# marcusrussi/approximateNN

Hardware: AMD Instinct MI355X
Metric: queries/sec, N=10M d=128 k=10 Q=10k float (query(): hash + candidate gather + L2 + top-k + refine) (higher is better)
Workload: dtype f32; 1 GPU; cfg3: N=10000000 d=128 k=10 tries=10 Q=10000/step float; streams=1, d_short=20, L1=6006, P1=4096, L2=110, P2=64, sum_par_maxes=286

## Files before the change

### approximatenn_amd/csrc/ann_host.hip

```cpp
#include <hip/hip_fp16.h>
#include <hip/hip_runtime.h>
#include <math.h>
#include <stdio.h>
#include <stdlib.h>
#include <string.h>
#include <time.h>

#include <algorithm>
#include <limits>
#include <mutex>
#include <vector>

#include "../../include/algg.h"
#include "../../include/ann_hip.h"
#include "../../include/gpu_comp.h"
#include "ann_hostpool.h"
#include "ann_precomp_kernels.h"
#include "ann_query_kernels.h"
#include "ann_probe_kernels.h"
#include "ann_recall_kernels.h"
#include "ann_exact_kernels.h"
#include "ann_filter_kernels.h"
#include "ann_tag_kernels.h"
#include "ann_kq_kernels.h"
// ... 202 lines not shown
static T *dev_alloc(size_t count) {
  void *p = NULL;
  HIPCHECK(hipMalloc(&p, (count ? count : 1) * sizeof(T)));
  return (T *)p;
}

static int device_cus() {
  static int cus[64] = {0};
  int dev = 0;
  if (hipGetDevice(&dev) != hipSuccess || dev < 0 || dev >= 64) return 256;
  if (!cus[dev]) {
    hipDeviceProp_t prop;
    cus[dev] = hipGetDeviceProperties(&prop, dev) == hipSuccess && prop.multiProcessorCount > 0 ? prop.multiProcessorCount : 256;
  }
  return cus[dev];
}

static unsigned grid_for(size_t work, unsigned block, unsigned cap = 1u << 20) {
  size_t g = (work + block - 1) / block;
  if (g < 1) g = 1;
  if (g > cap) g = cap;
  return (unsigned)g;
}

#define ANN_NCOUNTERS (8 + 64 * 8)
struct EventPair {
  hipEvent_t a, b;
};

struct annhip_workspace {
  DevBuf codes, cand_d, cand_i, nvt, nvo, top_i, top_d, flist, xids, xd, r2i, r2d, out_i, out_d;
  DevBuf pbits;
  DevBuf sorted;
  u32 *d_fcount = NULL;
  void release() {
    DevBuf *bufs[] = {&codes, &cand_d, &cand_i, &nvt, &nvo, &top_i, &top_d, &flist, &xids, &xd, &r2i, &r2d, &out_i, &out_d, &pbits, &sorted};
    for (DevBuf *b : bufs) b->release();
    if (d_fcount) HIPCHECK(hipFree(d_fcount));
    d_fcount = NULL;
  }
};

#ifdef USE_FLOAT
#define ANNHIP_ROWS_NARROW ANNHIP_ROWS_F16
#define ANN_NARROW_WHAT "binary16"
#else
#define ANNHIP_ROWS_NARROW ANNHIP_ROWS_F32
#define ANN_NARROW_WHAT "binary32"
#endif

struct annhip_index {
  size_t n = 0, k = 0, d = 0, ds = 0, lo = 0, hi = 0;
  int T = 0;
  FT *d_points = NULL;
  bool own_points = false;
  std::vector<u32 *> d_tabs;
  std::vector<uint2 *> d_segs;
  std::vector<uint4 *> d_segx;
  int use_seg = 1;
  std::vector<TryInfo> h_tries;
  TryInfo *d_tries = NULL;
  u32 *d_graph = NULL;
  FT *d_means = NULL, *d_bases = NULL;
  FT *d_graph_dists = NULL;
  u32 L1 = 0, P1 = 0, Lc1 = 0, L2 = 0, P2 = 0, Lc2 = 0;
  size_t sum_pm = 0;
  hipStream_t stream = 0;
  annhip_workspace ws;
  DevBuf io_y, io_ids, io_dist;
// ... 855 lines not shown
        constexpr bool FU = decltype(fu)::value, RG = decltype(rg)::value;
        using RT = typename decltype(rt)::type;
        allow_lds(stage1_select_kernel<D, SG, FU, RT, RG>, smem);
        for (size_t a = 0; a < Q; a += per) {
          QParams Pp = P;
          Pp.q0 = (u32)a, Pp.qn = (u32)std::min(per, Q - a);
          hipLaunchKernelGGL((stage1_select_kernel<D, SG, FU, RT, RG>), dim3(std::min<unsigned>(Pp.qn, max_grid)), dim3(64 * W), smem,
                             s, Pp, kq, y, alias, codes, K1, cap, runs_used, cand_d, cand_i, nvt, nvo, F, cand_key);
        }
      };
      auto launch = [&](auto sg, auto fu) {
        if constexpr (sel_regs_layout<decltype(dd)::value>()) {
          if (regs) return launch_sel(sg, fu, std::true_type{});
        } else if (regs) {
          die("launch_stage1: register selection chosen for a layout without one");
        }
        launch_sel(sg, fu, std::false_type{});
      };
      if (use_seg == 2) launch(Int<2>{}, std::false_type{});
      else if (use_seg && F.enabled == 1) launch(Int<1>{}, std::true_type{});
      else if (use_seg) launch(Int<1>{}, std::false_type{});
      else if (F.enabled == 1) launch(Int<0>{}, std::true_type{});
      else launch(Int<0>{}, std::false_type{});
    });
  });
  HIPCHECK(hipGetLastError());
  if (prof) s1_prof_end(ix, ev, Q, nvo, s);
  if (ix) ix->s1_launches += 1;
}

#ifdef USE_FLOAT
static void launch_prune_rescore(annhip_index *ix, const QParams &P, size_t Q, const FT *y, int kp, const FT *pre_d,
                                 const u32 *pre_i, const u32 *nvt, u32 *nvo, u32 *top_i, FT *top_d, u32 *fl, u32 *d_fcount,
                                 hipStream_t s) {
  if (!Q) return;
  if (kp < P.k + 1 || kp > ANN_PRUNE_KMAX || P.k + 1 > 32) die("launch_prune_rescore: preselection size out of range");
  PruneArgs A = {};
  A.points = P.points, A.y = y, A.pre_d = pre_d, A.pre_i = pre_i, A.nv_tot = nvt, A.nv_own = nvo;
  A.top_id = top_i, A.top_dist = top_d, A.flist = fl, A.fcount = d_fcount;
  A.exact_total = ix->d_rows + 2, A.uncertified = ix->d_rows + 4;
  A.E = ix->prune_E;
  A.n = P.n, A.Q = (u32)Q, A.L1 = P.L1, A.P1 = P.P1;
  A.d = P.d, A.k = P.k, A.Kp = kp;
  const dim3 grid((unsigned)((Q + ANN_PRUNE_WAVES - 1) / ANN_PRUNE_WAVES)), block(64 * ANN_PRUNE_WAVES);
  with_value(QueryLayouts{}, layout_code(P.d), [&](auto dc) {
    constexpr int D = decltype(dc)::value;
    if constexpr (D != 0 && !OcCode<D>::GEN) hipLaunchKernelGGL(prune_rescore_kernel<D>, grid, block, 0, s, A);
    else die("launch_prune_rescore: no register layout for this row length");
  });
  HIPCHECK(hipGetLastError());
}
#endif

static void launch_codes_probe(const QParams &P, size_t Q, const FT *y, u32 *codes, unsigned char *pbits, int pb, hipStream_t s,
                               u32 *zero_me = NULL) {
  const int wpb = ANN_PROBE_WPB;
  const size_t items = Q * (size_t)P.T;
  if (!items) return;
  if (pb < 1 || pb > P.ds || P.ds > 31) die("launch_codes_probe: pair bits outside 1..d_short");
  if (d_is_fast(P.d) && (size_t)P.d * sizeof(FT) <= 512 && env().codes_lpq) {
    const size_t smem = sizeof(FT) * ((size_t)P.ds + 1) * P.d + sizeof(u32) * ANN_WAVE * ANN_LPQ_WAVES +
                        sizeof(UB) * (size_t)P.ds * ANN_WAVE;
    const dim3 grid((unsigned)((Q + ANN_WAVE - 1) / ANN_WAVE), (unsigned)P.T);
    with_value(Pow2Layouts{}, layout_code(P.d, false), [&](auto dd) {
      constexpr int D = decltype(dd)::value;
      if constexpr (D > 0 && D * sizeof(FT) <= 512) {
        allow_lds(codes_probe_lpq_kernel<D>, smem);
        hipLaunchKernelGGL(codes_probe_lpq_kernel<D>, grid, dim3(64 * ANN_LPQ_WAVES), smem, s, P, (int)Q, y, codes, zero_me, pb, pbits);
      }
    });
  } else if (d_is_fast(P.d)) {
    const size_t smem = sizeof(FT) * (size_t)P.ds * P.d;
    const dim3 grid((unsigned)((Q + ANN_CODES_QPB - 1) / ANN_CODES_QPB), (unsigned)P.T);
// ... 136 lines not shown
  const unsigned block = len <= 128 ? 128 : 256;
  const unsigned flat = live_rows ? split : 0;
  const dim3 grid = live_rows ? dim3((unsigned)std::min<size_t>(nq * split, 512)) : dim3((unsigned)nq, split);
  with_value(QueryLayouts{}, layout_code(P.d), [&](auto dd) {
    with_rows(P, [&](auto rt) {
      constexpr int D = decltype(dd)::value;
      using RT = typename decltype(rt)::type;
      allow_lds(row_dists_kernel<D, MODE, RT>, smem);
      hipLaunchKernelGGL((row_dists_kernel<D, MODE, RT>), grid, dim3(block), smem, s, P, kq, y, alias, codes, qidx, xbase, len,
                         top_i, top_d, ids, dist, rows_done, live_rows, (u32)nq, chunk, live_off, flat);
    });
  });
  HIPCHECK(hipGetLastError());
}

static void launch_exact_select(u32 L, u32 len, u32 in_stride, int k, size_t nq, u32 *ids, FT *dist,
                                const u32 *qidx, u32 xbase, u32 *out_i, FT *out_d, int ostride, int ooff,
                                hipStream_t s, const u32 *live_rows = NULL, size_t *out64 = NULL, unsigned max_block = 1024,
                                u32 live_off = 0, TieArgs tie = TieArgs{NULL, NULL, 0, NULL, 0}) {
  if (!nq) return;
  const int lk = ann_lg(L);
  unsigned npairs = 8u << (lk > 4 ? lk - 4 : 0);
  if (live_rows) max_block = std::min(max_block, 256u);
  unsigned block = npairs >= max_block ? max_block : ((npairs + 63) / 64) * 64;
  if (block < 64) block = 64;
  const size_t row_smem = (size_t)len * (sizeof(FT) + sizeof(u32));
  const unsigned grid = live_rows ? (unsigned)std::min<size_t>(nq, 128) : (unsigned)nq;
  const bool in_lds = row_smem <= env().lds_row_max;
  const u32 Pn = (u32)1 << lk;
  int nw = 0;
  if ((tie.cand_d || tie.derive) && env().tie && L >= 16 && tie.K1 == k + 1 && tie.K1 <= ANN_WAVE && (u32)k <= Pn)
    nw = Pn <= 4096 ? 1 : Pn <= 8192 ? 2 : Pn <= 16384 ? 4 : 0;
  size_t tie_smem = nw ? ann_tie_lds_bytes(nw) : 0;
  if (nw && !tie.cand_d) tie_smem += ann_tie_derive_bytes(Pn);
  if (tie_smem > 150 * 1024) nw = 0;
  if (!nw) tie = TieArgs{NULL, NULL, 0, NULL, 0}, tie_smem = 0;
  const size_t smem = std::max(in_lds ? row_smem : (size_t)0, tie_smem);
  auto launch = [&](auto lds, auto nwc) {
    constexpr bool LDS = decltype(lds)::value;
    constexpr int NW = decltype(nwc)::value;
    allow_lds((exact_select_kernel<LDS, NW>), smem);
    hipLaunchKernelGGL((exact_select_kernel<LDS, NW>), dim3(grid), dim3(block), smem, s, L, len, in_stride, k, ids, dist, qidx,
                       xbase, out_i, out_d, ostride, ooff, live_rows, (u32)nq, out64, live_off, tie);
  };
  with_value(Ints<0, 1, 2, 4>{}, nw, [&](auto nwc) {
    if (in_lds) launch(std::true_type{}, nwc);
    else launch(std::false_type{}, nwc);
  });
  HIPCHECK(hipGetLastError());
}

template <typename IdOut>
static void launch_stage2_fused(const QParams &P, size_t Q, const FT *y, int alias, u32 xbase, size_t nq, const u32 *top_i,
                                const FT *top_d, IdOut *out_ids, FT *out_d, unsigned long long *rows_ctr, hipStream_t s) {
  if (!nq) return;
  size_t smem = sizeof(Key) * (size_t)P.k + 3 * sizeof(u32) * (size_t)P.Lc2 + 16;
  smem = (smem + 15) & ~(size_t)15;
  smem += sizeof(FT) * (size_t)P.Lc2;
  smem = (smem + 15) & ~(size_t)15;
  if (d_needs_lds_row(P.d)) smem += sizeof(FT) * (size_t)P.d * 3;
  with_value(QueryLayouts{}, layout_code(P.d), [&](auto dd) {
    with_rows(P, [&](auto rt) {
      constexpr int D = decltype(dd)::value;
      using RT = typename decltype(rt)::type;
      allow_lds((stage2_fused_kernel<D, IdOut, RT>), smem);
      hipLaunchKernelGGL((stage2_fused_kernel<D, IdOut, RT>), dim3((unsigned)nq), dim3(env().s2_threads), smem, s, P, (int)Q, y,
                         alias, top_i, top_d, P.Lc2, out_ids, out_d, rows_ctr, xbase);
// ... 36 lines not shown
        if (filter) {
          allow_lds((stage2_filter_kernel<D, TT, RT>), smem);
          hipLaunchKernelGGL((stage2_filter_kernel<D, TT, RT>), dim3((unsigned)nq), dim3(64 * W), smem, s, P, (int)Q, y, alias,
                             top_i, top_d, filter, P2, K1, cap, out, out_d, fl, d_fcount, exact_total, rows_ctr, xbase);
          return;
        }
        allow_lds((stage2_select_kernel<D, TT, RT>), smem);
        hipLaunchKernelGGL((stage2_select_kernel<D, TT, RT>), dim3((unsigned)nq), dim3(64 * W), smem, s, P, (int)Q, y, alias,
                           top_i, top_d, P2, K1, cap, out, out_d, fl, d_fcount, exact_total, rows_ctr, xbase);
      };
      if (out64) launch(out64);
      else launch(out32);
    });
  });
  HIPCHECK(hipGetLastError());
  if (P.fixed) return true;
  const size_t R = std::min(nq, chunk);
  u32 *ri = (u32 *)r2i.need(sizeof(u32) * R * P.Lc2);
  FT *rd = (FT *)r2d.need(sizeof(FT) * R * P.Lc2);
  for (size_t p0 = 0; p0 < nq; p0 += R) {
    const size_t np = std::min(R, nq - p0);
    launch_rows<MODE_GRAPH>(P, Q, y, alias, NULL, fl + p0, 0, np, P.Lc2, top_i, top_d, ri, rd, rows_ctr, s, d_fcount, (u32)p0);
    launch_exact_select(P.L2, P.Lc2, P.Lc2, P.k, np, ri, rd, fl + p0, 0, out32, out_d, P.k, 0, s, d_fcount, out64, 1024,
                        (u32)p0);
  }
  return true;
}

static long finalize_and_fallback(annhip_index *ix, const QParams &P, size_t Q, const FT *y, int alias,
                                  const u32 *codes, int mode, const FT *cand_d, const u32 *cand_i,
                                  const u32 *nvt, u32 *top_i, FT *top_d, int ostride, int ooff, DevBuf &flist,
                                  DevBuf &xids, DevBuf &xd, u32 *d_fcount, unsigned long long *rows_done,
                                  unsigned long long *exact_total, bool device_driven, hipStream_t s, size_t qstride = 0,
                                  bool prefinalized = false) {
  const int K1 = P.k + 1;
  unsigned long long *tie_ctr = ix ? ix->d_rows + 3 : NULL;
  const TieArgs tie0 = cand_d ? TieArgs{cand_d, cand_i, K1, tie_ctr, 0} : TieArgs{NULL, NULL, K1, tie_ctr, 1};
  u32 nflag = 0;
  u32 *fl = (u32 *)flist.need(sizeof(u32) * Q);
  const size_t row_bytes = (size_t)P.Lc1 * (sizeof(FT) + sizeof(u32));
  size_t chunk = env().exact_bytes / (row_bytes ? row_bytes : 1);
  if (chunk < 1) chunk = 1;
  if (mode == 0) {
    if (!prefinalized) {
      zero_u32_kernel<<<1, 1, 0, s>>>(d_fcount);
      hipLaunchKernelGGL(finalize1_kernel, dim3(grid_for(Q, 256, 1u << 30)), dim3(256), 0, s, (int)Q, P.k, K1, P.L1,
                         P.P1, cand_d, cand_i, nvt, top_i, top_d, ostride, ooff, fl, d_fcount, exact_total);
      HIPCHECK(hipGetLastError());
    }
    if (device_driven && Q <= 8 * chunk) {
      const size_t R = std::min(Q, chunk);
      u32 *ids = (u32 *)xids.need(sizeof(u32) * R * P.Lc1);
      FT *dist = (FT *)xd.need(sizeof(FT) * R * P.Lc1);
      for (size_t p0 = 0; p0 < Q; p0 += R) {
        const size_t nq = std::min(R, Q - p0);
        launch_rows<MODE_TABLE>(P, Q, y, alias, codes, fl + p0, 0, nq, P.Lc1, NULL, NULL, ids, dist, rows_done, s, d_fcount,
                                (u32)p0, qstride);
        launch_exact_select(P.L1, P.Lc1, P.Lc1, P.k, nq, ids, dist, fl + p0, 0, top_i, top_d, ostride, ooff, s, d_fcount,
                            NULL, 1024, (u32)p0, tie0);
      }
      return -1;
    }
    HIPCHECK(hipMemcpyAsync(&nflag, d_fcount, sizeof(u32), hipMemcpyDeviceToHost, s));
    HIPCHECK(hipStreamSynchronize(s));
  } else {
    nflag = (u32)Q;
    if (exact_total) {
      unsigned long long add = Q, cur = 0;
      HIPCHECK(hipMemcpyAsync(&cur, exact_total, sizeof cur, hipMemcpyDeviceToHost, s));
      HIPCHECK(hipStreamSynchronize(s));
// ... 131 lines not shown
      FusedTail F{1, P.Lc2, ids_dev, out_d, fl, ws.d_fcount, ix->d_rows + 2, NULL, NULL};
      cand_d = (FT *)ws.cand_d.need(sizeof(FT) * Q * K1);
      cand_i = (u32 *)ws.cand_i.need(sizeof(u32) * Q * K1);
      launch_stage1(ix, P, Q, y, alias, codes, cand_d, cand_i, NULL, nvo, s, ix->h_tries, ix->use_seg, F);
      seg_mark(ix, marks, s);
      unsigned long long *rows_ctr = ix->profile == 1 ? ix->d_rows + 8 : NULL;
      u32 *xi = (u32 *)ws.xids.need(sizeof(u32) * Q * P.Lc1);
      FT *xd = (FT *)ws.xd.need(sizeof(FT) * Q * P.Lc1);
      launch_rows<MODE_TABLE>(P, Q, y, alias, codes, fl, 0, Q, P.Lc1, NULL, NULL, xi, xd, rows_ctr, s, ws.d_fcount);
      launch_exact_select(P.L1, P.Lc1, P.Lc1, k, Q, xi, xd, fl, 0, top_i, top_d, k, 0, s, ws.d_fcount, NULL, 1024, 0,
                          TieArgs{cand_d, cand_i, K1, ix->d_rows + 3, 0});
      seg_mark(ix, marks, s);
      u32 *r2i = (u32 *)ws.r2i.need(sizeof(u32) * Q * P.Lc2);
      FT *r2d = (FT *)ws.r2d.need(sizeof(FT) * Q * P.Lc2);
      launch_rows<MODE_GRAPH>(P, Q, y, alias, NULL, fl, 0, Q, P.Lc2, top_i, top_d, r2i, r2d, rows_ctr, s, ws.d_fcount);
      seg_mark(ix, marks, s);
      launch_exact_select(P.L2, P.Lc2, P.Lc2, k, Q, r2i, r2d, fl, 0, NULL, out_d, k, 0, s, ws.d_fcount, ids_dev);
      seg_mark(ix, marks, s);
      seg_mark(ix, marks, s);
      if (marks) ix->seg_used.push_back(marks_store);
      ix->queries += (double)Q;
      return -1;
    }
  }
  bool prefinalized = false;
#ifdef USE_FLOAT
  if (pruned) {
    const int kp = ix->prune_kp;
    FT *pre_d = (FT *)ws.cand_d.need(sizeof(FT) * Q * kp);
    u32 *pre_i = (u32 *)ws.cand_i.need(sizeof(u32) * Q * kp);
    nvt = (u32 *)ws.nvt.need(sizeof(u32) * Q);
    u32 *nvo = (u32 *)ws.nvo.need(sizeof(u32) * Q);
    u32 *fl = (u32 *)ws.flist.need(sizeof(u32) * Q);
    prefinalized = true;
    if (!fcount_zeroed) zero_u32_kernel<<<1, 1, 0, s>>>(ws.d_fcount);
    QParams Pn = P;
    Pn.points_h = ix->d_points_h;
    EventPair ev;
    if (ix->profile) ev = s1_prof_begin(ix, s);
    launch_stage1(ix, Pn, Q, y, alias, codes, pre_d, pre_i, nvt, nvo, s, ix->h_tries, ix->use_seg,
                  FusedTail{0, 0, NULL, NULL, NULL, NULL, NULL, NULL, NULL}, NULL, 1, env().s1_slots, qstride, kp, false);
    launch_prune_rescore(ix, P, Q, y, kp, pre_d, pre_i, nvt, nvo, top_i, top_d, fl, ws.d_fcount, s);
    if (ix->profile) s1_prof_end(ix, ev, Q, nvo, s);
  } else
#endif
  if (mode == 0) {
    cand_d = (FT *)ws.cand_d.need(sizeof(FT) * Q * K1);
    cand_i = (u32 *)ws.cand_i.need(sizeof(u32) * Q * K1);
    nvt = (u32 *)ws.nvt.need(sizeof(u32) * Q);
    u32 *nvo = (u32 *)ws.nvo.need(sizeof(u32) * Q);
    u32 *fl = (u32 *)ws.flist.need(sizeof(u32) * Q);
    prefinalized = env().fin_tail != 0;
    if (prefinalized && !fcount_zeroed) zero_u32_kernel<<<1, 1, 0, s>>>(ws.d_fcount);
    launch_stage1(ix, P, Q, y, alias, codes, cand_d, cand_i, nvt, nvo, s, ix->h_tries, ix->use_seg,
                  FusedTail{prefinalized ? 2 : 0, 0, NULL, NULL, fl, ws.d_fcount, ix->d_rows + 2, top_i, top_d}, NULL, 1,
                  env().s1_slots, qstride);
  }
  seg_mark(ix, marks, s);
  unsigned long long *rows_ctr = ix->profile == 1 ? ix->d_rows + 8 : NULL;
  long nflag = finalize_and_fallback(ix, P, Q, y, alias, codes, mode, cand_d, cand_i, nvt, top_i, top_d, k, 0,
                                     ws.flist, ws.xids, ws.xd, ws.d_fcount, rows_ctr, ix->d_rows + 2, true, s, qstride,
                                     prefinalized);
  seg_mark(ix, marks, s);
  FT *out_d = dists_dev ? reinterpret_cast<FT *>(dists_dev) : (FT *)ws.out_d.need(sizeof(FT) * Q * k);
  if (ix->lo == 0 && ix->hi == ix->n && P.Lc2 <= 1024 && env().tail != 0) {
    launch_stage2_fused<size_t>(P, Q, y, alias, 0, Q, top_i, top_d, ids_dev, out_d, rows_ctr, s);
    seg_mark(ix, marks, s);
    seg_mark(ix, marks, s);
    seg_mark(ix, marks, s);
    if (marks) ix->seg_used.push_back(marks_store);
    ix->queries += (double)Q;
    return nflag;
  }
  if (ix->lo == 0 && ix->hi == ix->n && env().tail != 0 &&
      stage2_select_with_fallback(P, Q, y, alias, 0, Q, top_i, top_d, NULL, ids_dev, out_d, ws.flist, ws.d_fcount, ws.r2i,
                                  ws.r2d, ix->d_rows + 2, rows_ctr, s)) {
    seg_mark(ix, marks, s);
    seg_mark(ix, marks, s);
    seg_mark(ix, marks, s);
    if (marks) ix->seg_used.push_back(marks_store);
    ix->queries += (double)Q;
    return nflag;
  }
  u32 *out_i = (u32 *)ws.out_i.need(sizeof(u32) * Q * k);
  const size_t row_bytes = (size_t)P.Lc2 * (sizeof(FT) + sizeof(u32));
  size_t chunk = ((size_t)2 << 30) / row_bytes;
  if (chunk < 1) chunk = 1;
  for (size_t q0 = 0; q0 < Q; q0 += chunk) {
    const size_t nq = std::min(chunk, Q - q0);
    u32 *r2i = (u32 *)ws.r2i.need(sizeof(u32) * nq * P.Lc2);
    FT *r2d = (FT *)ws.r2d.need(sizeof(FT) * nq * P.Lc2);
    launch_rows<MODE_GRAPH>(P, Q, y, alias, NULL, NULL, (u32)q0, nq, P.Lc2, top_i, top_d, r2i, r2d, rows_ctr, s);
    if (q0 + chunk >= Q) seg_mark(ix, marks, s);
    launch_exact_select(P.L2, P.Lc2, P.Lc2, k, nq, r2i, r2d, NULL, (u32)q0, out_i, out_d, k, 0, s);
  }
// ... 2050 lines not shown
```

### approximatenn_amd/csrc/ann_prune_kernels.h

```cpp
#pragma once
#include "ann_rerank_kernels.h"

#define ANN_PRUNE_WAVES 4
#define ANN_PRUNE_KMAX 64

struct PruneArgs {
  const FT *points, *y;
  const FT *pre_d;
  const u32 *pre_i;
  const u32 *nv_tot;
  u32 *nv_own;
  u32 *top_id;
  FT *top_dist;
  u32 *flist, *fcount;
  unsigned long long *exact_total, *uncertified;
  double E;
  u32 n, Q, L1, P1;
  int d, k, Kp;
};

template <int D>
__global__ __launch_bounds__(64 * ANN_PRUNE_WAVES) void prune_rescore_kernel(PruneArgs A) {
  __shared__ Key s_keys[ANN_PRUNE_WAVES][ANN_PRUNE_KMAX], s_sorted[ANN_PRUNE_WAVES][ANN_PRUNE_KMAX];
  __shared__ u32 s_ids[ANN_PRUNE_WAVES][ANN_PRUNE_KMAX];
  constexpr int C = RowChunks<D>::C;
  const int lane = lane_id(), w = threadIdx.x >> 6;
  const int d = A.d, k = A.k, K1 = A.k + 1, Kp = A.Kp;
  const u32 q = __builtin_amdgcn_readfirstlane(blockIdx.x * ANN_PRUNE_WAVES + w);
  if (q >= A.Q) return;
  Key *keys = s_keys[w], *sorted = s_sorted[w];
  u32 *ids = s_ids[w];
  const u32 myid = lane < Kp ? A.pre_i[(size_t)q * Kp + lane] : ANN_ID_NONE;
  const bool real = myid < A.n;
  const u64 rm = __ballot(real);
  const int m = __builtin_popcountll(rm);
  if (real) ids[mask_rank(rm)] = myid;
  const ExLanes<D> ln(d, lane);
  VT a[C];
  const FT *yq = A.y + (size_t)q * d;
#pragma unroll
  for (int c = 0; c < C; c++) {
    if constexpr (D > 0) a[c] = reinterpret_cast<const VT *>(yq)[ln.p + c * ln.oc];
    else a[c] = oc_load_chunk<D, false>(yq, ln.p + c * ln.oc, d);
  }
  wave_lds_sync();
  const FT *__restrict__ points = A.points;
  auto load = [&](VT(&b)[C], int r0, u32 &id) {
    const int r = r0 + ln.g;
    id = ids[(ln.valid && r < m) ? r : r0];
    const FT *rp = points + (size_t)id * d;
#pragma unroll
    for (int c = 0; c < C; c++) {
      if constexpr (D > 0) b[c] = reinterpret_cast<const VT *>(rp)[ln.p + c * ln.oc];
      else b[c] = oc_load_chunk<D, false>(rp, ln.p + c * ln.oc, d);
    }
  };
  auto score = [&](const VT(&b)[C], int r0, u32 id) {
    const FT dist = ex_reduce<D>(a, b, ln.oc, ln.p, d);
    if (ln.valid && r0 + ln.g < m && ln.p == 0) keys[r0 + ln.g] = key_make(dist, id);
  };
  if (m) {
    VT b0[C], b1[C];
    u32 i0 = 0, i1 = 0;
    load(b0, 0, i0);
    for (int r0 = 0; r0 < m; r0 += 2 * ln.rpw) {
      const int r1 = r0 + ln.rpw, r2 = r1 + ln.rpw;
      if (r1 < m) load(b1, r1, i1);
      score(b0, r0, i0);
      if (r1 < m) {
        if (r2 < m) load(b0, r2, i0);
        score(b1, r1, i1);
      }
    }
  }
  wave_lds_sync();
  const Key me = keys[lane < m ? lane : 0];
  int rank = 0;
  for (int t = 0; t < m; t++) rank += key_less(keys[t], me) ? 1 : 0;
  if (lane < m) sorted[rank] = me;
  wave_lds_sync();
  const int me_cnt = m < K1 ? m : K1;
  bool cert = m < Kp;
  if (!cert && m >= K1) {
    const double B = (double)A.pre_d[(size_t)q * Kp + Kp - 1];
    const double tau = (double)key_dist(sorted[K1 - 1]);
    const double g1 = 1.0 - 0x1p-16;
    const double r = sqrt(B * g1) - A.E;
    if (B >= 0x1p-100 && r > 0.0) {
      const double LB = (r * r) * g1 * (1.0 - 0x1p-40);
      if (LB > tau) cert = true;
    }
  }
  bool bad = me_cnt < k;
  for (int t = lane; t + 1 < me_cnt; t += ANN_WAVE)
    if (ft_bits(key_dist(sorted[t])) == ft_bits(key_dist(sorted[t + 1]))) bad = true;
  if (me_cnt >= k && !(key_dist(sorted[k - 1]) < ft_inf())) bad = true;
  if (A.L1 > A.P1 && A.nv_tot[q] >= A.P1) bad = true;
  if (!cert || __ballot(bad) != 0) {
    if (lane == 0) {
      A.flist[atomicAdd(A.fcount, 1u)] = q;
      if (A.exact_total) atomicAdd(A.exact_total, 1ull);
      if (!cert && A.uncertified) atomicAdd(A.uncertified, 1ull);
    }
  } else {
    for (int t = lane; t < k; t += ANN_WAVE) {
      A.top_id[(size_t)q * k + t] = key_id(sorted[t]);
      A.top_dist[(size_t)q * k + t] = key_dist(sorted[t]);
    }
  }
  if (lane == 0 && A.nv_own) A.nv_own[q] = (A.nv_own[q] + 1) / 2 + (u32)m;
}

__global__ __launch_bounds__(256) void prune_rowerr_kernel(size_t rows, int d, const FT *__restrict__ points,
                                                           const RN *__restrict__ narrow, unsigned long long *out) {
  const int lane = lane_id();
  const size_t wave = ((size_t)blockIdx.x * blockDim.x + threadIdx.x) >> 6, waves = ((size_t)gridDim.x * blockDim.x) >> 6;
  double worst = 0;
  bool broken = false;
  for (size_t r = wave; r < rows; r += waves) {
    double acc = 0;
    for (int z = lane; z < d; z += ANN_WAVE) {
      const double df = (double)points[r * d + z] - (double)narrow[r * d + z];
      acc += df * df;
    }
#pragma unroll
    for (int s = 32; s >= 1; s >>= 1) acc += __shfl_xor(acc, s);
    if (!(acc < __builtin_inf())) broken = true;
    else if (acc > worst) worst = acc;
  }
  if (lane == 0) {
    atomicMax(out, (unsigned long long)__builtin_bit_cast(unsigned long long, worst));
    if (broken) atomicAdd(out + 1, 1ull);
  }
}
```

### approximatenn_amd/csrc/ann_query_kernels.h

```cpp
#pragma once
#include <type_traits>

#include "ann_device.h"
#include "ann_tie.h"

#ifndef ANN_ROWS_INFLIGHT
#define ANN_ROWS_INFLIGHT 1
#endif

struct TryInfo {
  const u32 *tab;
  const uint2 *seg;
  const uint4 *segx;
  u32 pm;
  u32 off;
  u32 end;
  u32 magic;
};

struct QParams {
  const FT *points;
  const TryInfo *tries;
  const u32 *graph;
  const FT *means;
// ... 14 lines not shown
#define ANN_S1_PREFETCH_NARROW 3
#endif
#ifndef ANN_S1_PREFETCH_OC
#define ANN_S1_PREFETCH_OC 2
#endif

template <bool NT>
__device__ __forceinline__ VT load_row_chunk(const VT *p) {
  if constexpr (NT) {
    typedef FT native_vec __attribute__((ext_vector_type(ANN_VEC)));
    native_vec v = __builtin_nontemporal_load(reinterpret_cast<const native_vec *>(p));
    return __builtin_bit_cast(VT, v);
  } else {
    return *p;
  }
}

template <typename RT>
__device__ __forceinline__ const RT *q_rows(const QParams &P) {
  if constexpr (std::is_same<RT, FT>::value) return P.points;
  else return P.points_h;
}
template <typename RT, bool NT>
__device__ __forceinline__ typename RowRaw<RT>::T load_row_raw(const RT *row, int ci) {
  if constexpr (std::is_same<RT, FT>::value) {
    return load_row_chunk<NT>(reinterpret_cast<const VT *>(row) + ci);
  } else {
    typedef typename RowRaw<RT>::T R;
    const R *p = reinterpret_cast<const R *>(row) + ci;
    if constexpr (NT) return __builtin_nontemporal_load(p);
    else return *p;
  }
}

template <int D, bool NT, typename RT>
__device__ __forceinline__ typename RowRaw<RT>::T oc_load_chunk(const RT *row, int ci, int d) {
  if constexpr (OcCode<D>::UA) {
    typename RowRaw<RT>::T v;
    RT *o = reinterpret_cast<RT *>(&v);
#pragma unroll
    for (int j = 0; j < ANN_VEC; j++) {
      const int z = ci * ANN_VEC + j;
      o[j] = z < d ? (NT ? __builtin_nontemporal_load(row + z) : row[z]) : (RT)0;
    }
    return v;
  } else {
    return load_row_raw<RT, NT>(row, ci);
  }
}
template <int D>
__device__ __forceinline__ int oc_tree_len(int d) { return OcCode<D>::UA ? d : 0; }

#define ANN_CODES_QPB 64
template <int D>
__global__ __launch_bounds__(256) void codes_kernel(QParams P, int Q, const FT *__restrict__ y,
                                                    u32 *__restrict__ codes, u32 *__restrict__ zero_me) {
  extern __shared__ __attribute__((aligned(16))) unsigned char smem[];
  if (zero_me && blockIdx.x == 0 && blockIdx.y == 0 && threadIdx.x == 0) *zero_me = 0;
  const int lane = lane_id(), w = threadIdx.x >> 6, wpb = blockDim.x >> 6;
  if constexpr (D > 0) {
    typedef RowLay<D> L;
    const int t = blockIdx.y;
    const int q0 = blockIdx.x * ANN_CODES_QPB, q1 = min(Q, q0 + ANN_CODES_QPB);
    VT *rows = reinterpret_cast<VT *>(smem);
    const VT *src = reinterpret_cast<const VT *>(P.bases + (size_t)t * P.ds * D);
    for (int i = threadIdx.x; i < P.ds * (D / ANN_VEC); i += blockDim.x) rows[i] = src[i];
// ... 404 lines not shown
    }
    const Key key = key_make(v, id);
    const bool pass = act && z == 0 && key_less(key, S.tau);
    const u64 mm = __ballot(pass);
    if (mm) {
      if (pass) S.kbuf[S.kcnt + mask_rank(mm)] = key;
      S.kcnt += __popcll(mm);
      if (S.kcnt + rpw > S.cap) sel_shrink(S);
    }
  }
}

template <int D, typename RT = FT, typename ST = SelState>
__device__ __forceinline__ void gather_select(const QParams &P, const u32 *list, int cnt, int alias, u32 x,
                                              const VT (&a)[RowChunks<D>::C],
                                              const FT *yq, FT *scratch, ST &S, const FT *yrow = NULL) {
  const int lane = lane_id();
  const RT *rows = q_rows<RT>(P);
  typedef typename RowRaw<RT>::T RR;
  if constexpr (D > 0) {
    typedef RowLay<D> L;
    constexpr int PF = std::is_same<RT, FT>::value ? ANN_S1_PREFETCH : ANN_S1_PREFETCH_NARROW;
    const int p = lane % L::LPR, g = lane / L::LPR;
    RR buf[PF][L::C];
    u32 idb[PF];
#pragma unroll
    for (int s = 0; s < PF; s++) {
      const int first = s * L::RPW;
      idb[s] = 0;
      if (first < cnt) {
        idb[s] = list[first + g < cnt ? first + g : first];
        const RT *rp = rows + (size_t)(idb[s] - P.lo) * D;
#pragma unroll
        for (int c = 0; c < L::C; c++) buf[s][c] = load_row_raw<RT, true>(rp, p + c * L::LPR);
      }
    }
    for (int base = 0; base < cnt; base += PF * L::RPW) {
#pragma unroll
      for (int s = 0; s < PF; s++) {
        const int cur = base + s * L::RPW;
        if (cur < cnt) {
          const u32 id = idb[s];
          const bool act = cur + g < cnt && !(alias && id == x);
          const FT dist = row_reduce<D, ROW_SQDIFF>(a, buf[s]);
          const int nb = cur + PF * L::RPW;
          if (nb < cnt) {
            idb[s] = list[nb + g < cnt ? nb + g : nb];
            const RT *rp = rows + (size_t)(idb[s] - P.lo) * D;
#pragma unroll
            for (int c = 0; c < L::C; c++) buf[s][c] = load_row_raw<RT, true>(rp, p + c * L::LPR);
          }
          const Key key = key_make(dist, id);
          const bool pass = act && p == 0 && key_less(key, S.tau);
          sel_offer(S, key, pass, L::RPW);
        }
      }
    }
  } else if constexpr (OcCode<D>::FOLD > 0) {
    const FoldPlan fp(P.d);
    gather_fold<OcCode<D>::FOLD, RT>(P, fp, list, cnt, alias, x, yrow, S);
  } else if constexpr (D < 0 && !OcCode<D>::GEN) {
    constexpr int C = OcCode<D>::C, OC = OcCode<D>::OC;
    constexpr int PF = ANN_S1_PREFETCH_OC;
    const OcLanes<D> ol(P.d, lane);
    const int oc = ol.oc, rpw = ol.rpw, g = ol.g, p = ol.p;
    RR buf[PF][C];
    u32 idb[PF];
#pragma unroll
    for (int s = 0; s < PF; s++) {
      const int first = s * rpw;
      idb[s] = 0;
      if (first < cnt) {
        idb[s] = list[(ol.valid && first + g < cnt) ? first + g : first];
        const RT *rp = rows + (size_t)(idb[s] - P.lo) * P.d;
#pragma unroll
        for (int c = 0; c < C; c++) buf[s][c] = oc_load_chunk<D, OcCode<D>::NT_ROWS>(rp, p + c * oc, P.d);
      }
    }
    for (int base = 0; base < cnt; base += PF * rpw) {
#pragma unroll
      for (int s = 0; s < PF; s++) {
        const int cur = base + s * rpw;
        if (cur < cnt) {
// ... 41 lines not shown
    u32 id;
    if (j < (u32)k) {
      id = key_id(top[j]);
      t_dist[j] = key_dist(top[j]);
    } else {
      const u32 parent = key_id(top[j / k - 1]), z = j % k;
      id = parent < P.n ? P.graph[(size_t)parent * k + z] : (P.graph[z] | P.n);
      const bool ok = id < P.n && !(alias && id == x) && id >= P.lo && id < P.hi;
      if (ok) {
        const u32 pos = atomicAdd(cnt2p, 1u);
        t_slot[pos] = j;
        t_gid[pos] = id;
      } else {
        t_dist[j] = ft_inf();
      }
    }
    t_ids[j] = id;
  }
  __syncthreads();
  const int cnt2 = (int)*cnt2p;
  if constexpr (D > 0) {
    typedef RowLay<D> L;
    constexpr int U = (ANN_ROWS_INFLIGHT / L::C) > 0 ? (ANN_ROWS_INFLIGHT / L::C) : 1;
    const int p = lane % L::LPR, g = lane / L::LPR;
    for (int base0 = w * L::RPW; base0 < cnt2; base0 += W * L::RPW * U) {
      RR b[U][L::C];
#pragma unroll
      for (int u = 0; u < U; u++) {
        const int r = base0 + u * W * L::RPW + g;
        if (base0 + u * W * L::RPW < cnt2) {
          const u32 id = t_gid[r < cnt2 ? r : base0];
          const RT *rp = rows + (size_t)(id - P.lo) * D;
#pragma unroll
          for (int c = 0; c < L::C; c++) b[u][c] = load_row_raw<RT, true>(rp, p + c * L::LPR);
        }
      }
#pragma unroll
      for (int u = 0; u < U; u++) {
        const int r = base0 + u * W * L::RPW + g;
        if (base0 + u * W * L::RPW < cnt2) {
          const FT dist = row_reduce<D, ROW_SQDIFF>(a, b[u]);
          if (r < cnt2 && p == 0) t_dist[t_slot[r]] = dist;
        }
      }
    }
  } else if constexpr (D < 0 && !OcCode<D>::GEN) {
    constexpr int C = OcCode<D>::C, OC = OcCode<D>::OC;
    constexpr int U = C <= 2 ? 4 : 2;
    const OcLanes<D> ol(P.d, lane);
    const int oc = ol.oc, rpw = ol.rpw, g = ol.g, p = ol.p;
    for (int base0 = w * rpw; base0 < cnt2; base0 += W * rpw * U) {
      RR b[U][C];
#pragma unroll
      for (int u = 0; u < U; u++) {
        const int r = base0 + u * W * rpw + g;
        if (base0 + u * W * rpw < cnt2) {
          const u32 id = t_gid[(ol.valid && r < cnt2) ? r : base0];
          const RT *rp = rows + (size_t)(id - P.lo) * P.d;
#pragma unroll
          for (int c = 0; c < C; c++) b[u][c] = oc_load_chunk<D, OcCode<D>::NT_ROWS>(rp, p + c * oc, P.d);
        }
      }
#pragma unroll
      for (int u = 0; u < U; u++) {
        const int r = base0 + u * W * rpw + g;
        if (base0 + u * W * rpw < cnt2) {
          const FT dist = row_reduce_oc<C, ROW_SQDIFF, OC>(a, b[u], oc, p, oc_tree_len<D>(P.d));
// ... 760 lines not shown
          id = parent < P.n ? P.graph[(size_t)parent * k + z] : (P.graph[z] | P.n);
        }
      }
      if (!DIST_ONLY) ids_row[j] = id;
      if (given) {
        dist_row[j] = top_dist[(size_t)x * P.k + j];
      } else {
        const bool own = id < P.n && !(alias && id == x) && id >= P.lo && id < P.hi;
        if (own) {
          const u32 pos = atomicAdd(&lcount[0], 1u);
          lslot[pos] = j;
          lid[pos] = id;
        } else {
          dist_row[j] = ft_inf();
        }
      }
    }
    __syncthreads();
    const int cnt = (int)lcount[0];
    gathered += cnt;
    if constexpr (D > 0) {
      typedef RowLay<D> L;
      constexpr int U = (ANN_ROWS_INFLIGHT / L::C) > 0 ? (ANN_ROWS_INFLIGHT / L::C) : 1;
      const int p = lane % L::LPR, g = lane / L::LPR;
      for (int base0 = w * L::RPW; base0 < cnt; base0 += W * L::RPW * U) {
        RR b[U][L::C];
#pragma unroll
        for (int u = 0; u < U; u++) {
          const int r = base0 + u * W * L::RPW + g;
          if (base0 + u * W * L::RPW < cnt) {
            const u32 id = lid[r < cnt ? r : base0];
            const RT *rp = rows + (size_t)(id - P.lo) * D;
#pragma unroll
            for (int c = 0; c < L::C; c++) b[u][c] = load_row_raw<RT, true>(rp, p + c * L::LPR);
          }
        }
#pragma unroll
        for (int u = 0; u < U; u++) {
          const int r = base0 + u * W * L::RPW + g;
          if (base0 + u * W * L::RPW < cnt) {
            const FT dist = row_reduce<D, ROW_SQDIFF>(a, b[u]);
            if (r < cnt && p == 0) dist_row[lslot[r]] = dist;
          }
        }
      }
    } else if constexpr (D < 0 && !OcCode<D>::GEN) {
      constexpr int C = OcCode<D>::C, OC = OcCode<D>::OC;
      const OcLanes<D> ol(P.d, lane);
      const int oc = ol.oc, rpw = ol.rpw, g = ol.g, p = ol.p;
      for (int base = w * rpw; base < cnt; base += W * rpw) {
        const int r = base + g;
        const bool act = ol.valid && r < cnt;
        const u32 id = lid[act ? r : base];
        const RT *rp = rows + (size_t)(id - P.lo) * P.d;
        RR b[C];
#pragma unroll
        for (int c = 0; c < C; c++) b[c] = oc_load_chunk<D, OcCode<D>::NT_ROWS>(rp, p + c * oc, P.d);
        const FT dist = row_reduce_oc<C, ROW_SQDIFF, OC>(a, b, oc, p, oc_tree_len<D>(P.d));
        if (act && p == 0) dist_row[lslot[r]] = dist;
      }
    } else {
      FT *m = yq + (size_t)(1 + w) * P.d;
      for (int r = w; r < cnt; r += W) {
        const u32 id = lid[r];
        const FT dist = row_reduce_generic<ROW_SQDIFF>(P.d, yq, rows + (size_t)(id - P.lo) * P.d, m);
        if (lane == 0) dist_row[lslot[r]] = dist;
      }
// ... 64 lines not shown
      }
    }
  }
  if (rows_done && threadIdx.x == 0) atomicAdd(&rows_done[(blockIdx.x & 63u) * 8u], (unsigned long long)cnt);
}

struct TieArgs {
  const FT *cand_d;
  const u32 *cand_i;
  int K1;
  unsigned long long *resolved;
  int derive;
};
template <bool USE_LDS, int NW>
__global__ __launch_bounds__(1024) void exact_select_kernel(u32 L, u32 len, u32 in_stride, int k,
                                                           u32 *__restrict__ ids_in,
                                                           FT *__restrict__ dist_in,
                                                           const u32 *__restrict__ qidx, u32 xbase,
                                                           u32 *__restrict__ out_id,
                                                           FT *__restrict__ out_dist, int ostride,
                                                           int ooff, const u32 *__restrict__ live_rows,
                                                           u32 nrows, size_t *__restrict__ out64, u32 live_off, TieArgs T) {
  extern __shared__ __attribute__((aligned(16))) unsigned char smem[];
  if (live_rows) nrows = min(nrows, max(*live_rows, live_off) - live_off);
  for (u32 row = blockIdx.x; row < nrows; row += gridDim.x) {
  const u32 x = qidx ? qidx[row] : xbase + row;
  u32 *gi = ids_in + (size_t)row * in_stride;
  FT *gd = dist_in + (size_t)row * in_stride;
  if constexpr (NW > 0) {
    if (T.cand_d || T.derive) {
      const size_t o = (size_t)x * ostride + ooff;
      const FT *cd = T.cand_d ? T.cand_d + (size_t)x * T.K1 : NULL;
      const u32 *ci = T.cand_d ? T.cand_i + (size_t)x * T.K1 : NULL;
      if (!T.cand_d && L >= 16 && T.K1 <= ANN_WAVE) {
        FT *dcd;
        u32 *dci;
        tie_derive_list((u32)1 << ann_lg(L), T.K1, gi, gd, smem + ann_tie_lds_bytes(NW), &dcd, &dci);
        cd = dcd, ci = dci;
      }
      const bool done = cd && tie_resolve<NW>(L, k, T.K1, gi, gd, cd, ci, smem,
                                              out64 ? NULL : out_id + o, out64 ? out64 + o : NULL, out_dist + o, T.resolved);
      if (done) {
        if (threadIdx.x == 0 && T.resolved) atomicAdd(T.resolved, 1ull);
        continue;
      }
    }
  }
  if (USE_LDS) {
    FT *sd = reinterpret_cast<FT *>(smem);
    u32 *si = reinterpret_cast<u32 *>(sd + len);
    for (u32 j = threadIdx.x; j < len; j += blockDim.x) sd[j] = gd[j], si[j] = gi[j];
    __syncthreads();
    block_topk_stage<true>(L, len, sd, si);
    for (int t = threadIdx.x; t < k; t += blockDim.x) {
      if (out64) out64[(size_t)x * ostride + ooff + t] = si[t];
      else out_id[(size_t)x * ostride + ooff + t] = si[t];
      out_dist[(size_t)x * ostride + ooff + t] = sd[t];
    }
  } else {
    block_topk_stage<false>(L, len, gd, gi);
    for (int t = threadIdx.x; t < k; t += blockDim.x) {
      if (out64) out64[(size_t)x * ostride + ooff + t] = gi[t];
      else out_id[(size_t)x * ostride + ooff + t] = gi[t];
      out_dist[(size_t)x * ostride + ooff + t] = gd[t];
    }
  }
  __syncthreads();
// ... 146 lines not shown
```

Measured before the change: 12.24 million queries/s.

## Pass pruned top-K1 lists to tie resolver and pick non-temporal row loads per layout

The prune-rescore kernel now writes its certified sorted top-(k+1) list into per-query tie buffers when it flags a query for fallback. The exact-select tie resolver can then use these lists directly instead of deriving them, and falls back to deriving only when a list is marked empty. The kernel is split into a per-wave device function, and the stage-1 row gathers use non-temporal loads only when a wave's load covers whole 128-byte lines, so binary16 rows at d=128 switch to normal loads. This adds global writes of the tie lists and extra buffers, and changes cache behaviour for the narrow-row gathers.

```diff
diff --git a/approximatenn_amd/csrc/ann_host.hip b/approximatenn_amd/csrc/ann_host.hip
--- a/approximatenn_amd/csrc/ann_host.hip
+++ b/approximatenn_amd/csrc/ann_host.hip
@@ -258,9 +258,10 @@
   DevBuf codes, cand_d, cand_i, nvt, nvo, top_i, top_d, flist, xids, xd, r2i, r2d, out_i, out_d;
   DevBuf pbits;
   DevBuf sorted;
+  DevBuf tie_d, tie_i;
   u32 *d_fcount = NULL;
   void release() {
-    DevBuf *bufs[] = {&codes, &cand_d, &cand_i, &nvt, &nvo, &top_i, &top_d, &flist, &xids, &xd, &r2i, &r2d, &out_i, &out_d, &pbits, &sorted};
+    DevBuf *bufs[] = {&codes, &cand_d, &cand_i, &nvt, &nvo, &top_i, &top_d, &flist, &xids, &xd, &r2i, &r2d, &out_i, &out_d, &pbits, &sorted, &tie_d, &tie_i};
     for (DevBuf *b : bufs) b->release();
     if (d_fcount) HIPCHECK(hipFree(d_fcount));
     d_fcount = NULL;
@@ -1182,13 +1183,14 @@
 #ifdef USE_FLOAT
 static void launch_prune_rescore(annhip_index *ix, const QParams &P, size_t Q, const FT *y, int kp, const FT *pre_d,
                                  const u32 *pre_i, const u32 *nvt, u32 *nvo, u32 *top_i, FT *top_d, u32 *fl, u32 *d_fcount,
-                                 hipStream_t s) {
+                                 FT *tie_d, u32 *tie_i, hipStream_t s) {
   if (!Q) return;
   if (kp < P.k + 1 || kp > ANN_PRUNE_KMAX || P.k + 1 > 32) die("launch_prune_rescore: preselection size out of range");
   PruneArgs A = {};
   A.points = P.points, A.y = y, A.pre_d = pre_d, A.pre_i = pre_i, A.nv_tot = nvt, A.nv_own = nvo;
   A.top_id = top_i, A.top_dist = top_d, A.flist = fl, A.fcount = d_fcount;
   A.exact_total = ix->d_rows + 2, A.uncertified = ix->d_rows + 4;
+  A.tie_d = tie_d, A.tie_i = tie_i;
   A.E = ix->prune_E;
   A.n = P.n, A.Q = (u32)Q, A.L1 = P.L1, A.P1 = P.P1;
   A.d = P.d, A.k = P.k, A.Kp = kp;
@@ -1391,7 +1393,7 @@
   if ((tie.cand_d || tie.derive) && env().tie && L >= 16 && tie.K1 == k + 1 && tie.K1 <= ANN_WAVE && (u32)k <= Pn)
     nw = Pn <= 4096 ? 1 : Pn <= 8192 ? 2 : Pn <= 16384 ? 4 : 0;
   size_t tie_smem = nw ? ann_tie_lds_bytes(nw) : 0;
-  if (nw && !tie.cand_d) tie_smem += ann_tie_derive_bytes(Pn);
+  if (nw && tie.derive) tie_smem += ann_tie_derive_bytes(Pn);
   if (tie_smem > 150 * 1024) nw = 0;
   if (!nw) tie = TieArgs{NULL, NULL, 0, NULL, 0}, tie_smem = 0;
   const size_t smem = std::max(in_lds ? row_smem : (size_t)0, tie_smem);
@@ -1494,10 +1496,10 @@
                                   const u32 *nvt, u32 *top_i, FT *top_d, int ostride, int ooff, DevBuf &flist,
                                   DevBuf &xids, DevBuf &xd, u32 *d_fcount, unsigned long long *rows_done,
                                   unsigned long long *exact_total, bool device_driven, hipStream_t s, size_t qstride = 0,
-                                  bool prefinalized = false) {
+                                  bool prefinalized = false, bool lists_may_be_empty = false) {
   const int K1 = P.k + 1;
   unsigned long long *tie_ctr = ix ? ix->d_rows + 3 : NULL;
-  const TieArgs tie0 = cand_d ? TieArgs{cand_d, cand_i, K1, tie_ctr, 0} : TieArgs{NULL, NULL, K1, tie_ctr, 1};
+  const TieArgs tie0 = cand_d ? TieArgs{cand_d, cand_i, K1, tie_ctr, lists_may_be_empty ? 1 : 0} : TieArgs{NULL, NULL, K1, tie_ctr, 1};
   u32 nflag = 0;
   u32 *fl = (u32 *)flist.need(sizeof(u32) * Q);
   const size_t row_bytes = (size_t)P.Lc1 * (sizeof(FT) + sizeof(u32));
@@ -1695,6 +1697,10 @@
     nvt = (u32 *)ws.nvt.need(sizeof(u32) * Q);
     u32 *nvo = (u32 *)ws.nvo.need(sizeof(u32) * Q);
     u32 *fl = (u32 *)ws.flist.need(sizeof(u32) * Q);
+#ifndef ANN_PRUNE_NO_TIE_LIST
+    cand_d = (FT *)ws.tie_d.need(sizeof(FT) * Q * K1);
+    cand_i = (u32 *)ws.tie_i.need(sizeof(u32) * Q * K1);
+#endif
     prefinalized = true;
     if (!fcount_zeroed) zero_u32_kernel<<<1, 1, 0, s>>>(ws.d_fcount);
     QParams Pn = P;
@@ -1703,7 +1709,7 @@
     if (ix->profile) ev = s1_prof_begin(ix, s);
     launch_stage1(ix, Pn, Q, y, alias, codes, pre_d, pre_i, nvt, nvo, s, ix->h_tries, ix->use_seg,
                   FusedTail{0, 0, NULL, NULL, NULL, NULL, NULL, NULL, NULL}, NULL, 1, env().s1_slots, qstride, kp, false);
-    launch_prune_rescore(ix, P, Q, y, kp, pre_d, pre_i, nvt, nvo, top_i, top_d, fl, ws.d_fcount, s);
+    launch_prune_rescore(ix, P, Q, y, kp, pre_d, pre_i, nvt, nvo, top_i, top_d, fl, ws.d_fcount, cand_d, cand_i, s);
     if (ix->profile) s1_prof_end(ix, ev, Q, nvo, s);
   } else
 #endif
@@ -1723,7 +1729,7 @@
   unsigned long long *rows_ctr = ix->profile == 1 ? ix->d_rows + 8 : NULL;
   long nflag = finalize_and_fallback(ix, P, Q, y, alias, codes, mode, cand_d, cand_i, nvt, top_i, top_d, k, 0,
                                      ws.flist, ws.xids, ws.xd, ws.d_fcount, rows_ctr, ix->d_rows + 2, true, s, qstride,
-                                     prefinalized);
+                                     prefinalized, pruned);
   seg_mark(ix, marks, s);
   FT *out_d = dists_dev ? reinterpret_cast<FT *>(dists_dev) : (FT *)ws.out_d.need(sizeof(FT) * Q * k);
   if (ix->lo == 0 && ix->hi == ix->n && P.Lc2 <= 1024 && env().tail != 0) {
diff --git a/approximatenn_amd/csrc/ann_prune_kernels.h b/approximatenn_amd/csrc/ann_prune_kernels.h
--- a/approximatenn_amd/csrc/ann_prune_kernels.h
+++ b/approximatenn_amd/csrc/ann_prune_kernels.h
@@ -14,35 +14,24 @@
   FT *top_dist;
   u32 *flist, *fcount;
   unsigned long long *exact_total, *uncertified;
+  FT *tie_d;
+  u32 *tie_i;
   double E;
   u32 n, Q, L1, P1;
   int d, k, Kp;
 };
 
 template <int D>
-__global__ __launch_bounds__(64 * ANN_PRUNE_WAVES) void prune_rescore_kernel(PruneArgs A) {
-  __shared__ Key s_keys[ANN_PRUNE_WAVES][ANN_PRUNE_KMAX], s_sorted[ANN_PRUNE_WAVES][ANN_PRUNE_KMAX];
-  __shared__ u32 s_ids[ANN_PRUNE_WAVES][ANN_PRUNE_KMAX];
+__device__ __forceinline__ void prune_rescore_wave(const PruneArgs &A, u32 q, const VT (&a)[RowChunks<D>::C], u32 myid, FT B,
+                                                   u32 vtot, u32 vown, Key *keys, Key *sorted, u32 *ids) {
   constexpr int C = RowChunks<D>::C;
-  const int lane = lane_id(), w = threadIdx.x >> 6;
+  const int lane = lane_id();
   const int d = A.d, k = A.k, K1 = A.k + 1, Kp = A.Kp;
-  const u32 q = __builtin_amdgcn_readfirstlane(blockIdx.x * ANN_PRUNE_WAVES + w);
-  if (q >= A.Q) return;
-  Key *keys = s_keys[w], *sorted = s_sorted[w];
-  u32 *ids = s_ids[w];
-  const u32 myid = lane < Kp ? A.pre_i[(size_t)q * Kp + lane] : ANN_ID_NONE;
   const bool real = myid < A.n;
   const u64 rm = __ballot(real);
   const int m = __builtin_popcountll(rm);
   if (real) ids[mask_rank(rm)] = myid;
   const ExLanes<D> ln(d, lane);
-  VT a[C];
-  const FT *yq = A.y + (size_t)q * d;
-#pragma unroll
-  for (int c = 0; c < C; c++) {
-    if constexpr (D > 0) a[c] = reinterpret_cast<const VT *>(yq)[ln.p + c * ln.oc];
-    else a[c] = oc_load_chunk<D, false>(yq, ln.p + c * ln.oc, d);
-  }
   wave_lds_sync();
   const FT *__restrict__ points = A.points;
   auto load = [&](VT(&b)[C], int r0, u32 &id) {
@@ -82,11 +71,11 @@
   const int me_cnt = m < K1 ? m : K1;
   bool cert = m < Kp;
   if (!cert && m >= K1) {
-    const double B = (double)A.pre_d[(size_t)q * Kp + Kp - 1];
+    const double Bd = (double)B;
     const double tau = (double)key_dist(sorted[K1 - 1]);
     const double g1 = 1.0 - 0x1p-16;
-    const double r = sqrt(B * g1) - A.E;
-    if (B >= 0x1p-100 && r > 0.0) {
+    const double r = sqrt(Bd * g1) - A.E;
+    if (Bd >= 0x1p-100 && r > 0.0) {
       const double LB = (r * r) * g1 * (1.0 - 0x1p-40);
       if (LB > tau) cert = true;
     }
@@ -95,12 +84,17 @@
   for (int t = lane; t + 1 < me_cnt; t += ANN_WAVE)
     if (ft_bits(key_dist(sorted[t])) == ft_bits(key_dist(sorted[t + 1]))) bad = true;
   if (me_cnt >= k && !(key_dist(sorted[k - 1]) < ft_inf())) bad = true;
-  if (A.L1 > A.P1 && A.nv_tot[q] >= A.P1) bad = true;
+  if (A.L1 > A.P1 && vtot >= A.P1) bad = true;
   if (!cert || __ballot(bad) != 0) {
     if (lane == 0) {
       A.flist[atomicAdd(A.fcount, 1u)] = q;
       if (A.exact_total) atomicAdd(A.exact_total, 1ull);
       if (!cert && A.uncertified) atomicAdd(A.uncertified, 1ull);
+    }
+    if (A.tie_d && lane < K1) {
+      const bool have = cert && lane < me_cnt;
+      A.tie_d[(size_t)q * K1 + lane] = have ? key_dist(sorted[lane]) : ft_inf();
+      A.tie_i[(size_t)q * K1 + lane] = have ? key_id(sorted[lane]) : ANN_ID_NONE;
     }
   } else {
     for (int t = lane; t < k; t += ANN_WAVE) {
@@ -108,7 +102,27 @@
       A.top_dist[(size_t)q * k + t] = key_dist(sorted[t]);
     }
   }
-  if (lane == 0 && A.nv_own) A.nv_own[q] = (A.nv_own[q] + 1) / 2 + (u32)m;
+  if (lane == 0 && A.nv_own) A.nv_own[q] = (vown + 1) / 2 + (u32)m;
+}
+
+template <int D>
+__global__ __launch_bounds__(64 * ANN_PRUNE_WAVES) void prune_rescore_kernel(PruneArgs A) {
+  __shared__ Key s_keys[ANN_PRUNE_WAVES][ANN_PRUNE_KMAX], s_sorted[ANN_PRUNE_WAVES][ANN_PRUNE_KMAX];
+  __shared__ u32 s_ids[ANN_PRUNE_WAVES][ANN_PRUNE_KMAX];
+  const int lane = lane_id(), w = threadIdx.x >> 6;
+  const u32 q = __builtin_amdgcn_readfirstlane(blockIdx.x * ANN_PRUNE_WAVES + w);
+  if (q >= A.Q) return;
+  const ExLanes<D> ln(A.d, lane);
+  VT a[RowChunks<D>::C];
+  const FT *yq = A.y + (size_t)q * A.d;
+#pragma unroll
+  for (int c = 0; c < RowChunks<D>::C; c++) {
+    if constexpr (D > 0) a[c] = reinterpret_cast<const VT *>(yq)[ln.p + c * ln.oc];
+    else a[c] = oc_load_chunk<D, false>(yq, ln.p + c * ln.oc, A.d);
+  }
+  const u32 myid = lane < A.Kp ? A.pre_i[(size_t)q * A.Kp + lane] : ANN_ID_NONE;
+  prune_rescore_wave<D>(A, q, a, myid, A.pre_d[(size_t)q * A.Kp + A.Kp - 1], A.nv_tot[q], A.nv_own ? A.nv_own[q] : 0u, s_keys[w],
+                        s_sorted[w], s_ids[w]);
 }
 
 __global__ __launch_bounds__(256) void prune_rowerr_kernel(size_t rows, int d, const FT *__restrict__ points,
diff --git a/approximatenn_amd/csrc/ann_query_kernels.h b/approximatenn_amd/csrc/ann_query_kernels.h
--- a/approximatenn_amd/csrc/ann_query_kernels.h
+++ b/approximatenn_amd/csrc/ann_query_kernels.h
@@ -70,6 +70,26 @@
     else return *p;
   }
 }
+template <int D, typename RT>
+constexpr bool row_loads_nt() {
+#ifdef ANN_S1_NARROW_NT
+  if (!std::is_same<RT, FT>::value) return ANN_S1_NARROW_NT != 0;
+#endif
+  return (RowLay<D>::LPR * (int)sizeof(typename RowRaw<RT>::T)) % 128 == 0;
+}
+#ifndef ANN_S1_NARROW_NT
+#ifdef USE_FLOAT
+static_assert(row_loads_nt<128, FT>() && !row_loads_nt<128, RN>(), "d = 128: native rows by whole lines, binary16 rows by halves");
+static_assert(row_loads_nt<64, FT>() && !row_loads_nt<64, RN>() && row_loads_nt<32, FT>() && !row_loads_nt<32, RN>(),
+              "d = 32, 64: 8 lanes per row, 128 bytes of a native row and 64 of a binary16 one per instruction");
+static_assert(row_loads_nt<256, FT>() && row_loads_nt<256, RN>(), "d = 256: 16 lanes per row, whole lines either way");
+#else
+static_assert(row_loads_nt<128, FT>() && row_loads_nt<128, RN>() && row_loads_nt<256, FT>() && row_loads_nt<256, RN>(),
+              "f64 library, d = 128, 256: 16 / 32 lanes per row, whole lines of native and of binary32 rows");
+static_assert(row_loads_nt<64, FT>() && !row_loads_nt<64, RN>() && row_loads_nt<32, FT>() && !row_loads_nt<32, RN>(),
+              "f64 library, d = 32, 64: 8 lanes per row, 128 bytes of a native row and 64 of a binary32 one per instruction");
+#endif
+#endif
 
 template <int D, bool NT, typename RT>
 __device__ __forceinline__ typename RowRaw<RT>::T oc_load_chunk(const RT *row, int ci, int d) {
@@ -540,7 +560,7 @@
         idb[s] = list[first + g < cnt ? first + g : first];
         const RT *rp = rows + (size_t)(idb[s] - P.lo) * D;
 #pragma unroll
-        for (int c = 0; c < L::C; c++) buf[s][c] = load_row_raw<RT, true>(rp, p + c * L::LPR);
+        for (int c = 0; c < L::C; c++) buf[s][c] = load_row_raw<RT, row_loads_nt<D, RT>()>(rp, p + c * L::LPR);
       }
     }
     for (int base = 0; base < cnt; base += PF * L::RPW) {
@@ -556,7 +576,7 @@
             idb[s] = list[nb + g < cnt ? nb + g : nb];
             const RT *rp = rows + (size_t)(idb[s] - P.lo) * D;
 #pragma unroll
-            for (int c = 0; c < L::C; c++) buf[s][c] = load_row_raw<RT, true>(rp, p + c * L::LPR);
+            for (int c = 0; c < L::C; c++) buf[s][c] = load_row_raw<RT, row_loads_nt<D, RT>()>(rp, p + c * L::LPR);
           }
           const Key key = key_make(dist, id);
           const bool pass = act && p == 0 && key_less(key, S.tau);
@@ -664,7 +684,7 @@
           const u32 id = t_gid[r < cnt2 ? r : base0];
           const RT *rp = rows + (size_t)(id - P.lo) * D;
 #pragma unroll
-          for (int c = 0; c < L::C; c++) b[u][c] = load_row_raw<RT, true>(rp, p + c * L::LPR);
+          for (int c = 0; c < L::C; c++) b[u][c] = load_row_raw<RT, row_loads_nt<D, RT>()>(rp, p + c * L::LPR);
         }
       }
 #pragma unroll
@@ -1491,7 +1511,7 @@
             const u32 id = lid[r < cnt ? r : base0];
             const RT *rp = rows + (size_t)(id - P.lo) * D;
 #pragma unroll
-            for (int c = 0; c < L::C; c++) b[u][c] = load_row_raw<RT, true>(rp, p + c * L::LPR);
+            for (int c = 0; c < L::C; c++) b[u][c] = load_row_raw<RT, row_loads_nt<D, RT>()>(rp, p + c * L::LPR);
           }
         }
 #pragma unroll
@@ -1622,7 +1642,9 @@
       const size_t o = (size_t)x * ostride + ooff;
       const FT *cd = T.cand_d ? T.cand_d + (size_t)x * T.K1 : NULL;
       const u32 *ci = T.cand_d ? T.cand_i + (size_t)x * T.K1 : NULL;
-      if (!T.cand_d && L >= 16 && T.K1 <= ANN_WAVE) {
+      const bool empty = !T.cand_d || (T.derive && ci[0] == ANN_ID_NONE);
+      if (empty) cd = NULL;
+      if (empty && T.derive && L >= 16 && T.K1 <= ANN_WAVE) {
         FT *dcd;
         u32 *dci;
         tie_derive_list((u32)1 << ann_lg(L), T.K1, gi, gd, smem + ann_tie_lds_bytes(NW), &dcd, &dci);
```

Result: faster. 13.38 million queries/s, median of 6 (+9.3%).
